# edenartlab/sd-lora-trainer

Measured on AMD Instinct MI355X. Metric: training images/sec, SDXL 1024px rank-16 LoRA, 1/2/4/8 GPU (job-parallel), higher is better.
Workload: dtype bf16

## Files before the change

sd-lora-trainer_amd/csrc/attn32.hip:

```cpp
#include "common.h"
#include "../../include/sdlt_kernels.h"
#include "attn32.h"

namespace {

constexpr float LOG2E = 1.4426950408889634f;
typedef float f32x16 __attribute__((ext_vector_type(16)));
constexpr int TILE = 64 * 128;

__device__ __forceinline__ int sw32(int row) { return (((row >> 1) & 1) << 2) | ((row >> 2) & 3); }
__device__ __forceinline__ int rmap(int rho) { return (rho & 0x13) | ((rho & 4) << 1) | ((rho & 8) >> 1); }

struct WgId { int x, y, z; };
__device__ __forceinline__ WgId xcd_wg() {
  const int gx = gridDim.x, gy = gridDim.y, n = gx * gy * gridDim.z;
  const int L = blockIdx.x + gx * (blockIdx.y + gy * blockIdx.z);
  const int k = L & 7, slot = L >> 3, q = n >> 3, r = n & 7;
  const int logical = (k < r ? k * (q + 1) : r * (q + 1) + (k - r) * q) + slot;
  WgId w;
  const int t = div_small_u(logical, gx);
  w.x = logical - t * gx;
  w.z = gridDim.z == 1 ? 0 : div_small_u(t, gy);
  w.y = t - w.z * gy;
  return w;
}

__device__ __forceinline__ void tile_dma(const bf16_t* src, int64_t ld, char* dst, int w2, int lane) {
#pragma unroll
  for (int pc = 0; pc < 4; ++pc) {
    const int piece = w2 * 4 + pc;
    const int r = piece * 8 + (lane >> 3);
    glds16(src + (int64_t)r * ld + (((lane & 7) ^ sw32(r)) << 3), dst + piece * 1024);
  }
}

template <int OFF>
__device__ __forceinline__ bf16x8 lds_b128(uint32_t a) {
  bf16x8 v;
  asm volatile("ds_read_b128 %0, %1 offset:%2" : "=v"(v) : "v"(a), "n"(OFF));
  return v;
}
template <int OFF>
__device__ __forceinline__ bf16x4 lds_tr(uint32_t a) {
  bf16x4 v;
  asm volatile("ds_read_b64_tr_b16 %0, %1 offset:%2" : "=v"(v) : "v"(a), "n"(OFF));
  return v;
}
template <int N>
__device__ __forceinline__ void wait_lgkm() { asm volatile("s_waitcnt lgkmcnt(%0)" ::"n"(N) : "memory"); }
__device__ __forceinline__ void pin(bf16x8& v) { asm volatile("" : "+v"(v)); }
__device__ __forceinline__ void pin(bf16x4& v) { asm volatile("" : "+v"(v)); }
template <int BLK>
__device__ __forceinline__ void rows_issue(bf16x8 (&f)[4], uint32_t tile, const int (&row)[4]) {
#pragma unroll
  for (int kk = 0; kk < 4; ++kk) f[kk] = lds_b128<BLK * 4096>(tile + row[kk]);
}
__device__ __forceinline__ void rows_pin(bf16x8 (&f)[4]) {
#pragma unroll
  for (int kk = 0; kk < 4; ++kk) pin(f[kk]);
}
struct TrFrag { bf16x4 v[4]; };
template <int CH>
__device__ __forceinline__ void tr_issue(TrFrag& f, uint32_t tile, const int (&t1)[2], const int (&t2)[2]) {
  f.v[0] = lds_tr<CH * 2048>(tile + t1[0]);
  f.v[1] = lds_tr<CH * 2048>(tile + t2[0]);
  f.v[2] = lds_tr<CH * 2048>(tile + t1[1]);
  f.v[3] = lds_tr<CH * 2048>(tile + t2[1]);
}
__device__ __forceinline__ void tr_pin(TrFrag& f) {
#pragma unroll
  for (int k = 0; k < 4; ++k) pin(f.v[k]);
}
__device__ __forceinline__ bf16x8 tr_get(const TrFrag& f, int db) { return __builtin_shufflevector(f.v[2 * db], f.v[2 * db + 1], 0, 1, 2, 3, 4, 5, 6, 7); }
__device__ __forceinline__ uint32_t lds_addr(const char* p) { return (uint32_t)(uintptr_t)(__attribute__((address_space(3))) const char*)p; }
__device__ __forceinline__ bf16x8 ld8(const bf16_t* p) {
  union { uint4 u; bf16x8 v; } c;
  c.u = *(const uint4*)p;
  return c.v;
}
__device__ __forceinline__ bf16x8 pack8v(const f32x16& v, int c2) {
  union { uint4 u; bf16x8 b; } c;
  c.u.x = pack2bf(v[8 * c2 + 0], v[8 * c2 + 1]); c.u.y = pack2bf(v[8 * c2 + 2], v[8 * c2 + 3]);
  c.u.z = pack2bf(v[8 * c2 + 4], v[8 * c2 + 5]); c.u.w = pack2bf(v[8 * c2 + 6], v[8 * c2 + 7]);
  return c.b;
}
__device__ __forceinline__ float half_max(float v) {
  auto r = __builtin_amdgcn_permlane32_swap(__float_as_uint(v), __float_as_uint(v), false, false);
  return fmaxf(__uint_as_float(r[0]), __uint_as_float(r[1]));
}
__device__ __forceinline__ float half_sum(float v) {
  auto r = __builtin_amdgcn_permlane32_swap(__float_as_uint(v), __float_as_uint(v), false, false);
  return __uint_as_float(r[0]) + __uint_as_float(r[1]);
}
#ifndef SDLT_A32_STORE16
#define SDLT_A32_STORE16 1
#endif
__device__ __forceinline__ void store_pair(bf16_t* p, int hl, uint2 ev, uint2 od) {
#if SDLT_A32_STORE16
  auto x = __builtin_amdgcn_permlane32_swap(ev.x, od.x, false, false);
  auto y = __builtin_amdgcn_permlane32_swap(ev.y, od.y, false, false);
  *(uint4*)p = make_uint4(x[0], y[0], x[1], y[1]);
#else
  *(uint2*)(p - 4 * hl) = ev;
  *(uint2*)(p - 4 * hl + 8) = od;
#endif
}

__device__ __forceinline__ void wait_dma_barrier() {
  asm volatile("s_waitcnt vmcnt(0)" ::: "memory");
  __syncthreads();
}

struct FragOff {
  int row[4];
  int t1[2], t2[2];
};
__device__ __forceinline__ FragOff frag_offsets(int lane) {
  FragOff f;
  const int hl = lane >> 5, c = lane & 31, rr = rmap(c);
#pragma unroll
  for (int kk = 0; kk < 4; ++kk) f.row[kk] = rr * 128 + (((2 * kk + hl) ^ sw32(rr)) << 4);
  const int g = lane >> 4, i = lane & 15;
  const int R = 8 * (g >> 1) + (i >> 2), swl = (((i >> 3) & 1) << 2) | ((g >> 1) << 1), chl = 2 * (g & 1) + ((i & 3) >> 1);
#pragma unroll
  for (int db = 0; db < 2; ++db) {
    f.t1[db] = R * 128 + (((4 * db + chl) ^ swl) << 4) + (i & 1) * 8;
    f.t2[db] = (R + 4) * 128 + (((4 * db + chl) ^ swl ^ 1) << 4) + (i & 1) * 8;
  }
  return f;
}

#define MFMA32(a, b, c) __builtin_amdgcn_mfma_f32_32x32x16_bf16(a, b, c, 0, 0, 0)

#ifndef SDLT_A32_DMA_SPLIT
#define SDLT_A32_DMA_SPLIT 1
#endif

#ifdef SDLT_ATTN32_TRACE
#define TR32_DECL(BUF_, ON_) long long* tr_ = (long long*)(BUF_); int tn_ = 0; const bool tron_ = (ON_) && tr_ != nullptr
#define TR32() do { if (tron_ && tn_ < 500) { __builtin_amdgcn_sched_barrier(0); tr_[tn_++] = clock64(); __builtin_amdgcn_sched_barrier(0); } } while (0)
#else
#define TR32_DECL(BUF_, ON_)
#define TR32() do { } while (0)
#endif

template <int KS>
__global__ __launch_bounds__(128 * KS) void attn32_fwd_kernel(const sdlt_attn_params p) {
  extern __shared__ __attribute__((aligned(16))) char smem[];
  const WgId wg = xcd_wg();
  const int b = wg.z, h = wg.y, q0 = wg.x * 64;
  const int lane = threadIdx.x & 63, wv = __builtin_amdgcn_readfirstlane(threadIdx.x >> 6);
  const int grp = wv >> 1, w2 = wv & 1, hl = lane >> 5, c = lane & 31;
  const int hc = h * 64;
  const int q = q0 + w2 * 32 + c;
  const bf16_t* Kb = (const bf16_t*)p.K + (int64_t)b * p.Nkp * p.ldk + hc;
  const bf16_t* Vb = (const bf16_t*)p.V + (int64_t)b * p.Nkp * p.ldv + hc;
  char* ring = smem + grp * (4 * TILE);
  const int ntile = p.Nk >> 6, niter = (ntile + KS - 1) / KS;
  if (grp < ntile) {
    tile_dma(Kb + (int64_t)grp * 64 * p.ldk, p.ldk, ring, w2, lane);
    tile_dma(Vb + (int64_t)grp * 64 * p.ldv, p.ldv, ring + TILE, w2, lane);
  }
  bf16x8 qf[4];
  {
    const bf16_t* qp = (const bf16_t*)p.Q + ((int64_t)b * p.Nqp + q) * p.ldq + hc + 8 * hl;
#pragma unroll
    for (int kk = 0; kk < 4; ++kk) qf[kk] = ld8(qp + 16 * kk);
  }
  const FragOff fo = frag_offsets(lane);
  float m = -1e30f, lsum = 0.f;
  f32x16 o[2];
#pragma unroll
  for (int db = 0; db < 2; ++db)
#pragma unroll
    for (int r = 0; r < 16; ++r) o[db][r] = 0.f;
  const float sl2 = p.scale * LOG2E;
  TR32_DECL(p.D, wg.x == 0 && wg.y == 0 && wg.z == 0 && threadIdx.x == 0);
  TR32();
  wait_dma_barrier();
  for (int it = 0; it < niter; ++it) {
    TR32();
    const int t = it * KS + grp;
    const char* Ks = ring + (it & 1) * (2 * TILE);
    const char* Vs = Ks + TILE;
    char* nb = ring + ((it + 1) & 1) * (2 * TILE);
    const bool more = t + KS < ntile;
#if SDLT_A32_DMA_SPLIT == 0
    if (more) {
      tile_dma(Kb + (int64_t)(t + KS) * 64 * p.ldk, p.ldk, nb, w2, lane);
      tile_dma(Vb + (int64_t)(t + KS) * 64 * p.ldv, p.ldv, nb + TILE, w2, lane);
    }
#endif
    TR32();
    if (t < ntile) {
      const uint32_t ka = lds_addr(Ks), va = lds_addr(Vs);
      bf16x8 k0f[4], k1f[4];
      TrFrag vt[4];
      rows_issue<0>(k0f, ka, fo.row);
      rows_issue<1>(k1f, ka, fo.row);
      tr_issue<0>(vt[0], va, fo.t1, fo.t2);
      tr_issue<1>(vt[1], va, fo.t1, fo.t2);
      f32x16 s[2];
#pragma unroll
      for (int blk = 0; blk < 2; ++blk)
#pragma unroll
        for (int r = 0; r < 16; ++r) s[blk][r] = 0.f;
      wait_lgkm<12>();
      rows_pin(k0f);
#pragma unroll
      for (int kk = 0; kk < 4; ++kk) s[0] = MFMA32(k0f[kk], qf[kk], s[0]);
#if SDLT_A32_DMA_SPLIT
      if (more) tile_dma(Kb + (int64_t)(t + KS) * 64 * p.ldk, p.ldk, nb, w2, lane);
#endif
      tr_issue<2>(vt[2], va, fo.t1, fo.t2);
      tr_issue<3>(vt[3], va, fo.t1, fo.t2);
      wait_lgkm<15>();
      rows_pin(k1f);
#pragma unroll
      for (int kk = 0; kk < 4; ++kk) s[1] = MFMA32(k1f[kk], qf[kk], s[1]);
#if SDLT_A32_DMA_SPLIT
      if (more) tile_dma(Vb + (int64_t)(t + KS) * 64 * p.ldv, p.ldv, nb + TILE, w2, lane);
#endif
      __builtin_amdgcn_sched_barrier(0);
      TR32();
      float tmax = s[0][0];
#pragma unroll
      for (int blk = 0; blk < 2; ++blk)
#pragma unroll
        for (int r = 0; r < 16; ++r) tmax = fmaxf(tmax, s[blk][r]);
      tmax = half_max(tmax);
      const float mn = fmaxf(m, tmax * sl2);
      const float alpha = __builtin_amdgcn_exp2f(m - mn);
      m = mn;
      float rs = 0.f;
#pragma unroll
      for (int blk = 0; blk < 2; ++blk)
#pragma unroll
        for (int r = 0; r < 16; ++r) {
          const float pv = __builtin_amdgcn_exp2f(__builtin_fmaf(s[blk][r], sl2, -mn));
          s[blk][r] = pv;
          rs += pv;
        }
      lsum = lsum * alpha + rs;
#pragma unroll
      for (int db = 0; db < 2; ++db)
#pragma unroll
        for (int r = 0; r < 16; ++r) o[db][r] *= alpha;
      __builtin_amdgcn_sched_barrier(0);
      TR32();
      wait_lgkm<0>();
#pragma unroll
      for (int ch = 0; ch < 4; ++ch) tr_pin(vt[ch]);
#pragma unroll
      for (int ch = 0; ch < 4; ++ch) {
        const bf16x8 pf = pack8v(s[ch >> 1], ch & 1);
#pragma unroll
        for (int db = 0; db < 2; ++db) o[db] = MFMA32(tr_get(vt[ch], db), pf, o[db]);
      }
    }
    TR32();
    wait_dma_barrier();
  }
  TR32();
  lsum = half_sum(lsum);
  if constexpr (KS > 1) {
    float* mg = (float*)smem + (((grp - 1) * 2 + w2) * 64 + lane) * 36;
    if (grp > 0) {
      mg[0] = m;
      mg[1] = lsum;
#pragma unroll
      for (int db = 0; db < 2; ++db)
#pragma unroll
        for (int j = 0; j < 4; ++j) *(f32x4*)(mg + 4 + db * 16 + j * 4) = (f32x4){o[db][4 * j], o[db][4 * j + 1], o[db][4 * j + 2], o[db][4 * j + 3]};
    }
    __syncthreads();
    if (grp > 0) return;
#pragma unroll
    for (int g2 = 1; g2 < KS; ++g2) {
      const float* sg = (const float*)smem + (((g2 - 1) * 2 + w2) * 64 + lane) * 36;
      const float m1 = sg[0], l1 = sg[1];
      const float mn = fmaxf(m, m1), a0 = __builtin_amdgcn_exp2f(m - mn), a1 = __builtin_amdgcn_exp2f(m1 - mn);
      m = mn;
      lsum = lsum * a0 + l1 * a1;
#pragma unroll
      for (int db = 0; db < 2; ++db)
#pragma unroll
        for (int j = 0; j < 4; ++j) {
          const f32x4 o1 = *(const f32x4*)(sg + 4 + db * 16 + j * 4);
#pragma unroll
          for (int r = 0; r < 4; ++r) o[db][4 * j + r] = o[db][4 * j + r] * a0 + o1[r] * a1;
        }
    }
  }
  const float inv = 1.f / lsum;
  if (hl == 0 && p.L) p.L[((int64_t)b * p.H + h) * p.Nq + q] = (m + log2f(lsum)) / LOG2E;
#ifndef SDLT_ATTN32_TRACE
  if (hl == 0 && p.D) p.D[((int64_t)b * p.H + h) * p.Nq + q] = 0.f;
#endif
  bf16_t* op = (bf16_t*)p.O + ((int64_t)b * p.Nqp + q) * p.ldo + hc + 8 * hl;
#pragma unroll
  for (int db = 0; db < 2; ++db)
#pragma unroll
    for (int jp = 0; jp < 2; ++jp) {
      uint2 w[2];
#pragma unroll
      for (int e = 0; e < 2; ++e) {
        const int j = 2 * jp + e;
        w[e].x = pack2bf(o[db][4 * j] * inv, o[db][4 * j + 1] * inv);
        w[e].y = pack2bf(o[db][4 * j + 2] * inv, o[db][4 * j + 3] * inv);
      }
      store_pair(op + 32 * db + 16 * jp, hl, w[0], w[1]);
    }
}

template <int KS>
__device__ __forceinline__ void attn32_dq_body(const sdlt_attn_params& p, char* smem, const int bx, const WgId wg) {
  const int b = wg.z, h = wg.y, q0 = bx * 64;
  const int lane = threadIdx.x & 63, wv = __builtin_amdgcn_readfirstlane(threadIdx.x >> 6);
  const int grp = wv >> 1, w2 = wv & 1, hl = lane >> 5, c = lane & 31;
  const int hc = h * 64;
  const int q = q0 + w2 * 32 + c;
  const bf16_t* Kb = (const bf16_t*)p.K + (int64_t)b * p.Nkp * p.ldk + hc;
  const bf16_t* Vb = (const bf16_t*)p.V + (int64_t)b * p.Nkp * p.ldv + hc;
  char* ring = smem + grp * (4 * TILE);
  const int ntile = p.Nk >> 6, niter = (ntile + KS - 1) / KS;
  if (grp < ntile) {
    tile_dma(Kb + (int64_t)grp * 64 * p.ldk, p.ldk, ring, w2, lane);
    tile_dma(Vb + (int64_t)grp * 64 * p.ldv, p.ldv, ring + TILE, w2, lane);
  }
  bf16x8 qf[4], gf[4];
  {
    const bf16_t* qp = (const bf16_t*)p.Q + ((int64_t)b * p.Nqp + q) * p.ldq + hc + 8 * hl;
    const bf16_t* gp = (const bf16_t*)p.dO + ((int64_t)b * p.Nqp + q) * p.lddo + hc + 8 * hl;
#pragma unroll
    for (int kk = 0; kk < 4; ++kk) {
      qf[kk] = ld8(qp + 16 * kk);
      gf[kk] = ld8(gp + 16 * kk);
    }
  }
  const float Lq = p.L[((int64_t)b * p.H + h) * p.Nq + q] * LOG2E;
  const float Dq = p.D[((int64_t)b * p.H + h) * p.Nq + q];
  const FragOff fo = frag_offsets(lane);
  f32x16 dq[2];
#pragma unroll
  for (int db = 0; db < 2; ++db)
#pragma unroll
    for (int r = 0; r < 16; ++r) dq[db][r] = 0.f;
  const float sl2 = p.scale * LOG2E;
  TR32_DECL(p.dK32, bx == 0 && wg.y == 0 && wg.z == 0 && threadIdx.x == 0);
  TR32();
  wait_dma_barrier();
  for (int it = 0; it < niter; ++it) {
    TR32();
    const int t = it * KS + grp;
    const char* Ks = ring + (it & 1) * (2 * TILE);
    const char* Vs = Ks + TILE;
    char* nb = ring + ((it + 1) & 1) * (2 * TILE);
    const bool more = t + KS < ntile;
#if SDLT_A32_DMA_SPLIT == 0
    if (more) {
      tile_dma(Kb + (int64_t)(t + KS) * 64 * p.ldk, p.ldk, nb, w2, lane);
      tile_dma(Vb + (int64_t)(t + KS) * 64 * p.ldv, p.ldv, nb + TILE, w2, lane);
    }
#endif
    TR32();
    if (t < ntile) {
      const uint32_t ka = lds_addr(Ks), va = lds_addr(Vs);
      bf16x8 kr[2][4], vr[2][4];
      TrFrag kt[2][2];
      rows_issue<0>(kr[0], ka, fo.row);
      rows_issue<0>(vr[0], va, fo.row);
      tr_issue<0>(kt[0][0], ka, fo.t1, fo.t2);
      tr_issue<1>(kt[0][1], ka, fo.t1, fo.t2);
#pragma unroll
      for (int blk = 0; blk < 2; ++blk) {
        f32x16 s, dp;
#pragma unroll
        for (int r = 0; r < 16; ++r) { s[r] = 0.f; dp[r] = 0.f; }
        wait_lgkm<8>();
        rows_pin(kr[blk]);
        rows_pin(vr[blk]);
#pragma unroll
        for (int kk = 0; kk < 4; ++kk) {
          s = MFMA32(kr[blk][kk], qf[kk], s);
          dp = MFMA32(vr[blk][kk], gf[kk], dp);
        }
        if (blk == 0) {
          rows_issue<1>(kr[1], ka, fo.row);
          rows_issue<1>(vr[1], va, fo.row);
        }
#if SDLT_A32_DMA_SPLIT
        if (more) {
          if (blk == 0) tile_dma(Kb + (int64_t)(t + KS) * 64 * p.ldk, p.ldk, nb, w2, lane);
          else tile_dma(Vb + (int64_t)(t + KS) * 64 * p.ldv, p.ldv, nb + TILE, w2, lane);
        }
#endif
        __builtin_amdgcn_sched_barrier(0);
        TR32();
#pragma unroll
        for (int r = 0; r < 16; ++r) {
          const float pv = __builtin_amdgcn_exp2f(__builtin_fmaf(s[r], sl2, -Lq));
          s[r] = pv * (dp[r] - Dq);
        }
        __builtin_amdgcn_sched_barrier(0);
        TR32();
        if (blk == 0) wait_lgkm<8>(); else wait_lgkm<0>();
        tr_pin(kt[blk][0]);
        tr_pin(kt[blk][1]);
#pragma unroll
        for (int c2 = 0; c2 < 2; ++c2) {
          const bf16x8 dsf = pack8v(s, c2);
#pragma unroll
          for (int db = 0; db < 2; ++db) dq[db] = MFMA32(tr_get(kt[blk][c2], db), dsf, dq[db]);
        }
        if (blk == 0) {
          tr_issue<2>(kt[1][0], ka, fo.t1, fo.t2);
          tr_issue<3>(kt[1][1], ka, fo.t1, fo.t2);
        }
        TR32();
      }
    }
    wait_dma_barrier();
  }
  TR32();
  if constexpr (KS > 1) {
    float* mg = (float*)smem + (((grp - 1) * 2 + w2) * 64 + lane) * 36;
    if (grp > 0) {
#pragma unroll
      for (int db = 0; db < 2; ++db)
#pragma unroll
        for (int j = 0; j < 4; ++j) *(f32x4*)(mg + db * 16 + j * 4) = (f32x4){dq[db][4 * j], dq[db][4 * j + 1], dq[db][4 * j + 2], dq[db][4 * j + 3]};
    }
    __syncthreads();
    if (grp > 0) return;
#pragma unroll
    for (int g2 = 1; g2 < KS; ++g2) {
      const float* sg = (const float*)smem + (((g2 - 1) * 2 + w2) * 64 + lane) * 36;
#pragma unroll
      for (int db = 0; db < 2; ++db)
#pragma unroll
        for (int j = 0; j < 4; ++j) {
          const f32x4 o1 = *(const f32x4*)(sg + db * 16 + j * 4);
#pragma unroll
          for (int r = 0; r < 4; ++r) dq[db][4 * j + r] += o1[r];
        }
    }
  }
  bf16_t* op = (bf16_t*)p.dQ + ((int64_t)b * p.Nqp + q) * p.lddq + hc + 8 * hl;
#pragma unroll
  for (int db = 0; db < 2; ++db)
#pragma unroll
    for (int jp = 0; jp < 2; ++jp) {
      uint2 w[2];
#pragma unroll
      for (int e = 0; e < 2; ++e) {
        const int j = 2 * jp + e;
        w[e].x = pack2bf(dq[db][4 * j] * p.scale, dq[db][4 * j + 1] * p.scale);
        w[e].y = pack2bf(dq[db][4 * j + 2] * p.scale, dq[db][4 * j + 3] * p.scale);
      }
      store_pair(op + 32 * db + 16 * jp, hl, w[0], w[1]);
    }
}

template <int KS>
__device__ __forceinline__ void attn32_dkdv_body(const sdlt_attn_params& p, char* smem, const int bx, const WgId wg) {
  constexpr int RING = 2 * (2 * TILE + 512);
  const int b = wg.z, h = wg.y, k0 = bx * 64;
  const int lane = threadIdx.x & 63, wv = __builtin_amdgcn_readfirstlane(threadIdx.x >> 6);
  const int grp = wv >> 1, w2 = wv & 1, hl = lane >> 5, c = lane & 31;
  const int hc = h * 64;
  const int key = k0 + w2 * 32 + c;
  const bf16_t* Qb = (const bf16_t*)p.Q + (int64_t)b * p.Nqp * p.ldq + hc;
  const bf16_t* Gb = (const bf16_t*)p.dO + (int64_t)b * p.Nqp * p.lddo + hc;
  const float* Lb = p.L + ((int64_t)b * p.H + h) * p.Nq;
  const float* Db = p.D + ((int64_t)b * p.H + h) * p.Nq;
  char* ring = smem + grp * RING;
  const int ntile = p.Nq >> 6, niter = (ntile + KS - 1) / KS;
  auto stage_q = [&](int t, char* buf) { tile_dma(Qb + (int64_t)t * 64 * p.ldq, p.ldq, buf, w2, lane); };
  auto stage_g = [&](int t, char* buf) {
    tile_dma(Gb + (int64_t)t * 64 * p.lddo, p.lddo, buf + TILE, w2, lane);
    if (lane < 16) glds16((w2 ? Db : Lb) + t * 64 + lane * 4, buf + 2 * TILE + w2 * 256);
  };
  auto stage = [&](int t, char* buf) { stage_q(t, buf); stage_g(t, buf); };
  if (grp < ntile) stage(grp, ring);
  bf16x8 kf[4], vf[4];
  {
    const bf16_t* kp = (const bf16_t*)p.K + ((int64_t)b * p.Nkp + key) * p.ldk + hc + 8 * hl;
    const bf16_t* vp = (const bf16_t*)p.V + ((int64_t)b * p.Nkp + key) * p.ldv + hc + 8 * hl;
#pragma unroll
    for (int kk = 0; kk < 4; ++kk) {
      kf[kk] = ld8(kp + 16 * kk);
      vf[kk] = ld8(vp + 16 * kk);
    }
  }
  const FragOff fo = frag_offsets(lane);
  f32x16 dk[2], dv[2];
#pragma unroll
  for (int db = 0; db < 2; ++db)
#pragma unroll
    for (int r = 0; r < 16; ++r) { dk[db][r] = 0.f; dv[db][r] = 0.f; }
  const float sl2 = p.scale * LOG2E;
  TR32_DECL(p.dK32 ? p.dK32 + 1024 : nullptr, bx == 0 && wg.y == 0 && wg.z == 0 && threadIdx.x == 0);
  TR32();
  wait_dma_barrier();
  for (int it = 0; it < niter; ++it) {
    TR32();
    const int t = it * KS + grp;
    const char* Qs = ring + (it & 1) * (2 * TILE + 512);
    const char* Gs = Qs + TILE;
    const float* Ls = (const float*)(Gs + TILE);
    const float* Ds = Ls + 64;
    char* nb = ring + ((it + 1) & 1) * (2 * TILE + 512);
    const bool more = t + KS < ntile;
#if SDLT_A32_DMA_SPLIT == 0
    if (more) stage(t + KS, nb);
#endif
    TR32();
    if (t < ntile) {
      const uint32_t qa = lds_addr(Qs), ga = lds_addr(Gs);
      bf16x8 qr[2][4], gr[2][4];
      TrFrag gt[2][2], qt[2][2];
      rows_issue<0>(qr[0], qa, fo.row);
      rows_issue<0>(gr[0], ga, fo.row);
      tr_issue<0>(gt[0][0], ga, fo.t1, fo.t2);
      tr_issue<0>(qt[0][0], qa, fo.t1, fo.t2);
#pragma unroll
      for (int blk = 0; blk < 2; ++blk) {
        f32x16 s, dp;
#pragma unroll
        for (int r = 0; r < 16; ++r) { s[r] = 0.f; dp[r] = 0.f; }
        wait_lgkm<8>();
        rows_pin(qr[blk]);
        rows_pin(gr[blk]);
#pragma unroll
        for (int kk = 0; kk < 4; ++kk) {
          s = MFMA32(qr[blk][kk], kf[kk], s);
          dp = MFMA32(gr[blk][kk], vf[kk], dp);
        }
        if (blk == 0) {
          tr_issue<1>(gt[0][1], ga, fo.t1, fo.t2);
          tr_issue<1>(qt[0][1], qa, fo.t1, fo.t2);
        } else {
          tr_issue<3>(gt[1][1], ga, fo.t1, fo.t2);
          tr_issue<3>(qt[1][1], qa, fo.t1, fo.t2);
        }
#if SDLT_A32_DMA_SPLIT
        if (more) {
          if (blk == 0) stage_q(t + KS, nb);
          else stage_g(t + KS, nb);
        }
#endif
        __builtin_amdgcn_sched_barrier(0);
        TR32();
#pragma unroll
        for (int c2 = 0; c2 < 2; ++c2) {
          const int qb = blk * 32 + c2 * 16 + 8 * hl;
          const f32x4 l0 = *(const f32x4*)(Ls + qb), l1 = *(const f32x4*)(Ls + qb + 4);
          const f32x4 d0 = *(const f32x4*)(Ds + qb), d1 = *(const f32x4*)(Ds + qb + 4);
#pragma unroll
          for (int e = 0; e < 8; ++e) {
            const float lq = (e < 4 ? l0[e & 3] : l1[e & 3]) * LOG2E, dd = e < 4 ? d0[e & 3] : d1[e & 3];
            const float pv = __builtin_amdgcn_exp2f(__builtin_fmaf(s[8 * c2 + e], sl2, -lq));
            s[8 * c2 + e] = pv;
            dp[8 * c2 + e] = pv * (dp[8 * c2 + e] - dd);
          }
        }
        __builtin_amdgcn_sched_barrier(0);
        TR32();
        wait_lgkm<8>();
        tr_pin(gt[blk][0]);
        tr_pin(qt[blk][0]);
        {
          const bf16x8 pf = pack8v(s, 0), dsf = pack8v(dp, 0);
#pragma unroll
          for (int db = 0; db < 2; ++db) {
            dv[db] = MFMA32(tr_get(gt[blk][0], db), pf, dv[db]);
            dk[db] = MFMA32(tr_get(qt[blk][0], db), dsf, dk[db]);
          }
        }
        if (blk == 0) {
          rows_issue<1>(qr[1], qa, fo.row);
          rows_issue<1>(gr[1], ga, fo.row);
          tr_issue<2>(gt[1][0], ga, fo.t1, fo.t2);
          tr_issue<2>(qt[1][0], qa, fo.t1, fo.t2);
          wait_lgkm<15>();
        } else {
          wait_lgkm<0>();
        }
        tr_pin(gt[blk][1]);
        tr_pin(qt[blk][1]);
        {
          const bf16x8 pf = pack8v(s, 1), dsf = pack8v(dp, 1);
#pragma unroll
          for (int db = 0; db < 2; ++db) {
            dv[db] = MFMA32(tr_get(gt[blk][1], db), pf, dv[db]);
            dk[db] = MFMA32(tr_get(qt[blk][1], db), dsf, dk[db]);
          }
        }
        TR32();
      }
    }
    wait_dma_barrier();
  }
  TR32();
  if constexpr (KS > 1) {
    float* mg = (float*)smem + (((grp - 1) * 2 + w2) * 64 + lane) * 68;
    if (grp > 0) {
#pragma unroll
      for (int db = 0; db < 2; ++db)
#pragma unroll
        for (int j = 0; j < 4; ++j) {
          *(f32x4*)(mg + db * 16 + j * 4) = (f32x4){dk[db][4 * j], dk[db][4 * j + 1], dk[db][4 * j + 2], dk[db][4 * j + 3]};
          *(f32x4*)(mg + 32 + db * 16 + j * 4) = (f32x4){dv[db][4 * j], dv[db][4 * j + 1], dv[db][4 * j + 2], dv[db][4 * j + 3]};
        }
    }
    __syncthreads();
    if (grp > 0) return;
#pragma unroll
    for (int g2 = 1; g2 < KS; ++g2) {
      const float* sg = (const float*)smem + (((g2 - 1) * 2 + w2) * 64 + lane) * 68;
#pragma unroll
      for (int db = 0; db < 2; ++db)
#pragma unroll
        for (int j = 0; j < 4; ++j) {
          const f32x4 a = *(const f32x4*)(sg + db * 16 + j * 4), e = *(const f32x4*)(sg + 32 + db * 16 + j * 4);
#pragma unroll
          for (int r = 0; r < 4; ++r) {
            dk[db][4 * j + r] += a[r];
            dv[db][4 * j + r] += e[r];
          }
        }
    }
  }
  const int64_t row = (int64_t)b * p.Nkp + key;
  bf16_t* kp2 = (bf16_t*)p.dK + row * p.lddk + hc + 8 * hl;
  bf16_t* vp2 = (bf16_t*)p.dV + row * p.lddv + hc + 8 * hl;
#pragma unroll
  for (int db = 0; db < 2; ++db)
#pragma unroll
    for (int jp = 0; jp < 2; ++jp) {
      uint2 wk[2], wv[2];
#pragma unroll
      for (int e = 0; e < 2; ++e) {
        const int j = 2 * jp + e;
        wk[e].x = pack2bf(dk[db][4 * j] * p.scale, dk[db][4 * j + 1] * p.scale);
        wk[e].y = pack2bf(dk[db][4 * j + 2] * p.scale, dk[db][4 * j + 3] * p.scale);
        wv[e].x = pack2bf(dv[db][4 * j], dv[db][4 * j + 1]);
        wv[e].y = pack2bf(dv[db][4 * j + 2], dv[db][4 * j + 3]);
      }
      store_pair(kp2 + 32 * db + 16 * jp, hl, wk[0], wk[1]);
      store_pair(vp2 + 32 * db + 16 * jp, hl, wv[0], wv[1]);
    }
}

template <int KS>
__global__ __launch_bounds__(128 * KS) void attn32_bwd_both_kernel(const sdlt_attn_params p) {
  extern __shared__ __attribute__((aligned(16))) char smem[];
  const int ndq = p.Nq >> 6;
  const WgId wg = xcd_wg();
  if (wg.x < ndq) attn32_dq_body<KS>(p, smem, wg.x, wg);
  else attn32_dkdv_body<KS>(p, smem, wg.x - ndq, wg);
}

template <typename F>
int set_smem32(F f, int bytes) { return sdlt_raise_smem((const void*)f, bytes); }

}

bool sdlt_attn32_ok(const sdlt_attn_params& p) {
  return p.d == 64 && !p.causal && p.Nq >= 64 && p.Nk >= 64 && (p.Nq % 64) == 0 && (p.Nk % 64) == 0 && p.Nqp >= p.Nq && p.Nkp >= p.Nk;
}

int sdlt_attn32_fwd(const sdlt_attn_params& p, int ks, hipStream_t s) {
  dim3 grid(p.Nq / 64, p.H, p.B);
#define FWD32(KS_)                                                                                           \
  do {                                                                                                       \
    const int sm = (KS_) * 4 * TILE;                                                                         \
    if (set_smem32(attn32_fwd_kernel<KS_>, sm)) SDLT_FAIL(SDLT_ERR_LAUNCH, "sdlt_attn32_fwd: LDS attribute"); \
    hipLaunchKernelGGL((attn32_fwd_kernel<KS_>), grid, dim3(128 * (KS_)), sm, s, p);                          \
  } while (0)
  if (ks >= 4) FWD32(4);
  else if (ks >= 2) FWD32(2);
  else FWD32(1);
  SDLT_CHECK_LAUNCH();
  return SDLT_OK;
}

int sdlt_attn32_bwd_both(const sdlt_attn_params& p, int ks, hipStream_t s) {
  dim3 grid(p.Nq / 64 + p.Nk / 64, p.H, p.B);
#define BWD32(KS_)                                                                                                 \
  do {                                                                                                             \
    const int sm = (KS_) * 2 * (2 * TILE + 512);                                                                   \
    if (set_smem32(attn32_bwd_both_kernel<KS_>, sm)) SDLT_FAIL(SDLT_ERR_LAUNCH, "sdlt_attn32_bwd: LDS attribute"); \
    hipLaunchKernelGGL((attn32_bwd_both_kernel<KS_>), grid, dim3(128 * (KS_)), sm, s, p);                           \
  } while (0)
  if (ks >= 4) BWD32(4);
  else if (ks >= 2) BWD32(2);
  else BWD32(1);
  SDLT_CHECK_LAUNCH();
  return SDLT_OK;
}
```

Baseline: 24.19.

## Interleave MFMA, softmax, LDS reads and DMA in attention backward kernels

Reschedules the dQ and dK/dV backward attention loops so the S and dP MFMAs, exp2 softmax, LDS fragment loads and per-piece global-to-LDS DMA are interleaved between fine-grained scheduling barriers, in place of running as separate phases. It folds the -D subtraction into the dP accumulator init, using a -D seed in dQ and a sign-flipped V with a negated dK scale in dK/dV. It also moves the L/D LDS reads into explicit early ds_read_b128 issues. The aim is to hide LDS and DMA latency behind matrix ops. The cost is more register pressure and a fragile hand schedule that relies on lgkm wait counts being correct.

Result: no change. 24.38, median of 6 (+0.8%).

```diff
diff --git a/sd-lora-trainer_amd/csrc/attn32.hip b/sd-lora-trainer_amd/csrc/attn32.hip
--- a/sd-lora-trainer_amd/csrc/attn32.hip
+++ b/sd-lora-trainer_amd/csrc/attn32.hip
@@ -313,6 +313,30 @@
     }
 }
 
+#define GAP32() __builtin_amdgcn_sched_barrier(0)
+
+template <int OFF>
+__device__ __forceinline__ f32x4 lds_f4(uint32_t a) {
+  f32x4 v;
+  asm volatile("ds_read_b128 %0, %1 offset:%2" : "=v"(v) : "v"(a), "n"(OFF));
+  return v;
+}
+__device__ __forceinline__ void pin(f32x4& v) { asm volatile("" : "+v"(v)); }
+template <int CH, int K>
+__device__ __forceinline__ void tr_issue1(TrFrag& f, uint32_t tile, const FragOff& fo) {
+  f.v[K] = lds_tr<CH * 2048>(tile + ((K & 1) ? fo.t2[K >> 1] : fo.t1[K >> 1]));
+}
+__device__ __forceinline__ void tile_dma1(const bf16_t* src, int64_t ld, char* dst, int w2, int lane, int pc) {
+  const int piece = w2 * 4 + pc;
+  const int r = piece * 8 + (lane >> 3);
+  glds16(src + (int64_t)r * ld + (((lane & 7) ^ sw32(r)) << 3), dst + piece * 1024);
+}
+__device__ __forceinline__ bf16x8 pk_frag(const uint32_t* pk) {
+  union { uint4 u; bf16x8 b; } c;
+  c.u = make_uint4(pk[0], pk[1], pk[2], pk[3]);
+  return c.b;
+}
+
 template <int KS>
 __device__ __forceinline__ void attn32_dq_body(const sdlt_attn_params& p, char* smem, const int bx, const WgId wg) {
   const int b = wg.z, h = wg.y, q0 = bx * 64;
@@ -338,8 +362,13 @@
       gf[kk] = ld8(gp + 16 * kk);
     }
   }
-  const float Lq = p.L[((int64_t)b * p.H + h) * p.Nq + q] * LOG2E;
-  const float Dq = p.D[((int64_t)b * p.H + h) * p.Nq + q];
+  const float nLq = -(p.L[((int64_t)b * p.H + h) * p.Nq + q] * LOG2E);
+  f32x16 nd;
+  {
+    const float Dq = p.D[((int64_t)b * p.H + h) * p.Nq + q];
+#pragma unroll
+    for (int r = 0; r < 16; ++r) nd[r] = -Dq;
+  }
   const FragOff fo = frag_offsets(lane);
   f32x16 dq[2];
 #pragma unroll
@@ -357,12 +386,6 @@
     const char* Vs = Ks + TILE;
     char* nb = ring + ((it + 1) & 1) * (2 * TILE);
     const bool more = t + KS < ntile;
-#if SDLT_A32_DMA_SPLIT == 0
-    if (more) {
-      tile_dma(Kb + (int64_t)(t + KS) * 64 * p.ldk, p.ldk, nb, w2, lane);
-      tile_dma(Vb + (int64_t)(t + KS) * 64 * p.ldv, p.ldv, nb + TILE, w2, lane);
-    }
-#endif
     TR32();
     if (t < ntile) {
       const uint32_t ka = lds_addr(Ks), va = lds_addr(Vs);
@@ -376,47 +399,58 @@
       for (int blk = 0; blk < 2; ++blk) {
         f32x16 s, dp;
 #pragma unroll
-        for (int r = 0; r < 16; ++r) { s[r] = 0.f; dp[r] = 0.f; }
-        wait_lgkm<8>();
+        for (int r = 0; r < 16; ++r) s[r] = 0.f;
+        if (blk == 0) wait_lgkm<8>(); else wait_lgkm<0>();
         rows_pin(kr[blk]);
         rows_pin(vr[blk]);
+        GAP32();
 #pragma unroll
         for (int kk = 0; kk < 4; ++kk) {
           s = MFMA32(kr[blk][kk], qf[kk], s);
-          dp = MFMA32(vr[blk][kk], gf[kk], dp);
-        }
-        if (blk == 0) {
-          rows_issue<1>(kr[1], ka, fo.row);
-          rows_issue<1>(vr[1], va, fo.row);
-        }
-#if SDLT_A32_DMA_SPLIT
-        if (more) {
-          if (blk == 0) tile_dma(Kb + (int64_t)(t + KS) * 64 * p.ldk, p.ldk, nb, w2, lane);
-          else tile_dma(Vb + (int64_t)(t + KS) * 64 * p.ldv, p.ldv, nb + TILE, w2, lane);
-        }
-#endif
-        __builtin_amdgcn_sched_barrier(0);
+          if (blk == 0) {
+            if (kk < 2) { kr[1][2 * kk] = lds_b128<4096>(ka + fo.row[2 * kk]); kr[1][2 * kk + 1] = lds_b128<4096>(ka + fo.row[2 * kk + 1]); }
+            else { vr[1][2 * kk - 4] = lds_b128<4096>(va + fo.row[2 * kk - 4]); vr[1][2 * kk - 3] = lds_b128<4096>(va + fo.row[2 * kk - 3]); }
+          } else {
+            if (kk == 0) { tr_issue1<2, 0>(kt[1][0], ka, fo); tr_issue1<2, 1>(kt[1][0], ka, fo); }
+            if (kk == 1) { tr_issue1<2, 2>(kt[1][0], ka, fo); tr_issue1<2, 3>(kt[1][0], ka, fo); }
+            if (kk == 2) { tr_issue1<3, 0>(kt[1][1], ka, fo); tr_issue1<3, 1>(kt[1][1], ka, fo); }
+            if (kk == 3) { tr_issue1<3, 2>(kt[1][1], ka, fo); tr_issue1<3, 3>(kt[1][1], ka, fo); }
+          }
+          GAP32();
+        }
         TR32();
 #pragma unroll
-        for (int r = 0; r < 16; ++r) {
-          const float pv = __builtin_amdgcn_exp2f(__builtin_fmaf(s[r], sl2, -Lq));
-          s[r] = pv * (dp[r] - Dq);
-        }
-        __builtin_amdgcn_sched_barrier(0);
+        for (int kk = 0; kk < 4; ++kk) {
+          dp = MFMA32(vr[blk][kk], gf[kk], kk == 0 ? nd : dp);
+#pragma unroll
+          for (int r = 4 * kk; r < 4 * kk + 4; ++r) s[r] = __builtin_amdgcn_exp2f(__builtin_fmaf(s[r], sl2, nLq));
+          if (more) {
+            if (blk == 0) tile_dma1(Kb + (int64_t)(t + KS) * 64 * p.ldk, p.ldk, nb, w2, lane, kk);
+            else tile_dma1(Vb + (int64_t)(t + KS) * 64 * p.ldv, p.ldv, nb + TILE, w2, lane, kk);
+          }
+          GAP32();
+        }
         TR32();
+#pragma unroll
+        for (int r = 0; r < 8; ++r) s[r] *= dp[r];
+        const bf16x8 ds0 = pack8v(s, 0);
         if (blk == 0) wait_lgkm<8>(); else wait_lgkm<0>();
         tr_pin(kt[blk][0]);
         tr_pin(kt[blk][1]);
-#pragma unroll
-        for (int c2 = 0; c2 < 2; ++c2) {
-          const bf16x8 dsf = pack8v(s, c2);
-#pragma unroll
-          for (int db = 0; db < 2; ++db) dq[db] = MFMA32(tr_get(kt[blk][c2], db), dsf, dq[db]);
-        }
-        if (blk == 0) {
-          tr_issue<2>(kt[1][0], ka, fo.t1, fo.t2);
-          tr_issue<3>(kt[1][1], ka, fo.t1, fo.t2);
-        }
+        GAP32();
+        dq[0] = MFMA32(tr_get(kt[blk][0], 0), ds0, dq[0]);
+#pragma unroll
+        for (int r = 8; r < 12; ++r) s[r] *= dp[r];
+        GAP32();
+        dq[1] = MFMA32(tr_get(kt[blk][0], 1), ds0, dq[1]);
+#pragma unroll
+        for (int r = 12; r < 16; ++r) s[r] *= dp[r];
+        GAP32();
+        const bf16x8 ds1 = pack8v(s, 1);
+        GAP32();
+        dq[0] = MFMA32(tr_get(kt[blk][1], 0), ds1, dq[0]);
+        dq[1] = MFMA32(tr_get(kt[blk][1], 1), ds1, dq[1]);
+        GAP32();
         TR32();
       }
     }
@@ -493,6 +527,13 @@
       vf[kk] = ld8(vp + 16 * kk);
     }
   }
+#pragma unroll
+  for (int kk = 0; kk < 4; ++kk) {
+    union { bf16x8 v; uint4 u; } n;
+    n.v = vf[kk];
+    n.u.x ^= 0x80008000u; n.u.y ^= 0x80008000u; n.u.z ^= 0x80008000u; n.u.w ^= 0x80008000u;
+    vf[kk] = n.v;
+  }
   const FragOff fo = frag_offsets(lane);
   f32x16 dk[2], dv[2];
 #pragma unroll
@@ -508,18 +549,23 @@
     const int t = it * KS + grp;
     const char* Qs = ring + (it & 1) * (2 * TILE + 512);
     const char* Gs = Qs + TILE;
-    const float* Ls = (const float*)(Gs + TILE);
-    const float* Ds = Ls + 64;
     char* nb = ring + ((it + 1) & 1) * (2 * TILE + 512);
     const bool more = t + KS < ntile;
-#if SDLT_A32_DMA_SPLIT == 0
-    if (more) stage(t + KS, nb);
-#endif
     TR32();
     if (t < ntile) {
       const uint32_t qa = lds_addr(Qs), ga = lds_addr(Gs);
+      const uint32_t la = lds_addr(Gs + TILE) + 32 * hl, da = la + 256;
       bf16x8 qr[2][4], gr[2][4];
       TrFrag gt[2][2], qt[2][2];
+      f32x4 lv[2][4], dd[2][4];
+#define LD_ISSUE(BLK_)                                                                  \
+  do {                                                                                  \
+    lv[BLK_][0] = lds_f4<(BLK_) * 128>(la);      lv[BLK_][1] = lds_f4<(BLK_) * 128 + 16>(la); \
+    lv[BLK_][2] = lds_f4<(BLK_) * 128 + 64>(la); lv[BLK_][3] = lds_f4<(BLK_) * 128 + 80>(la); \
+    dd[BLK_][0] = lds_f4<(BLK_) * 128>(da);      dd[BLK_][1] = lds_f4<(BLK_) * 128 + 16>(da); \
+    dd[BLK_][2] = lds_f4<(BLK_) * 128 + 64>(da); dd[BLK_][3] = lds_f4<(BLK_) * 128 + 80>(da); \
+  } while (0)
+      LD_ISSUE(0);
       rows_issue<0>(qr[0], qa, fo.row);
       rows_issue<0>(gr[0], ga, fo.row);
       tr_issue<0>(gt[0][0], ga, fo.t1, fo.t2);
@@ -527,78 +573,81 @@
 #pragma unroll
       for (int blk = 0; blk < 2; ++blk) {
         f32x16 s, dp;
-#pragma unroll
-        for (int r = 0; r < 16; ++r) { s[r] = 0.f; dp[r] = 0.f; }
+        float lq[16];
         wait_lgkm<8>();
         rows_pin(qr[blk]);
         rows_pin(gr[blk]);
 #pragma unroll
+        for (int j = 0; j < 4; ++j) { pin(lv[blk][j]); pin(dd[blk][j]); }
+#pragma unroll
+        for (int r = 0; r < 16; ++r) { s[r] = 0.f; dp[r] = dd[blk][r >> 2][r & 3]; }
+        GAP32();
+#pragma unroll
         for (int kk = 0; kk < 4; ++kk) {
           s = MFMA32(qr[blk][kk], kf[kk], s);
+#pragma unroll
+          for (int r = 4 * kk; r < 4 * kk + 4; ++r) lq[r] = lv[blk][kk][r & 3] * LOG2E;
+          gt[blk][1].v[kk] = blk == 0 ? lds_tr<2048>(ga + ((kk & 1) ? fo.t2[kk >> 1] : fo.t1[kk >> 1])) : lds_tr<3 * 2048>(ga + ((kk & 1) ? fo.t2[kk >> 1] : fo.t1[kk >> 1]));
+          GAP32();
+        }
+#pragma unroll
+        for (int kk = 0; kk < 4; ++kk) {
           dp = MFMA32(gr[blk][kk], vf[kk], dp);
-        }
-        if (blk == 0) {
-          tr_issue<1>(gt[0][1], ga, fo.t1, fo.t2);
-          tr_issue<1>(qt[0][1], qa, fo.t1, fo.t2);
-        } else {
-          tr_issue<3>(gt[1][1], ga, fo.t1, fo.t2);
-          tr_issue<3>(qt[1][1], qa, fo.t1, fo.t2);
-        }
-#if SDLT_A32_DMA_SPLIT
-        if (more) {
-          if (blk == 0) stage_q(t + KS, nb);
-          else stage_g(t + KS, nb);
-        }
-#endif
-        __builtin_amdgcn_sched_barrier(0);
+#pragma unroll
+          for (int r = 4 * kk; r < 4 * kk + 4; ++r) s[r] = __builtin_amdgcn_exp2f(__builtin_fmaf(s[r], sl2, -lq[r]));
+          qt[blk][1].v[kk] = blk == 0 ? lds_tr<2048>(qa + ((kk & 1) ? fo.t2[kk >> 1] : fo.t1[kk >> 1])) : lds_tr<3 * 2048>(qa + ((kk & 1) ? fo.t2[kk >> 1] : fo.t1[kk >> 1]));
+          if (more) {
+            if (blk == 0) tile_dma1(Qb + (int64_t)(t + KS) * 64 * p.ldq, p.ldq, nb, w2, lane, kk);
+            else tile_dma1(Gb + (int64_t)(t + KS) * 64 * p.lddo, p.lddo, nb + TILE, w2, lane, kk);
+          }
+          GAP32();
+        }
+        if (more && blk == 1 && lane < 16) glds16((w2 ? Db : Lb) + (t + KS) * 64 + lane * 4, nb + 2 * TILE + w2 * 256);
         TR32();
 #pragma unroll
-        for (int c2 = 0; c2 < 2; ++c2) {
-          const int qb = blk * 32 + c2 * 16 + 8 * hl;
-          const f32x4 l0 = *(const f32x4*)(Ls + qb), l1 = *(const f32x4*)(Ls + qb + 4);
-          const f32x4 d0 = *(const f32x4*)(Ds + qb), d1 = *(const f32x4*)(Ds + qb + 4);
-#pragma unroll
-          for (int e = 0; e < 8; ++e) {
-            const float lq = (e < 4 ? l0[e & 3] : l1[e & 3]) * LOG2E, dd = e < 4 ? d0[e & 3] : d1[e & 3];
-            const float pv = __builtin_amdgcn_exp2f(__builtin_fmaf(s[8 * c2 + e], sl2, -lq));
-            s[8 * c2 + e] = pv;
-            dp[8 * c2 + e] = pv * (dp[8 * c2 + e] - dd);
-          }
-        }
-        __builtin_amdgcn_sched_barrier(0);
-        TR32();
+        for (int r = 0; r < 8; ++r) dp[r] *= s[r];
+        const bf16x8 pf0 = pack8v(s, 0), dsf0 = pack8v(dp, 0);
         wait_lgkm<8>();
         tr_pin(gt[blk][0]);
         tr_pin(qt[blk][0]);
-        {
-          const bf16x8 pf = pack8v(s, 0), dsf = pack8v(dp, 0);
-#pragma unroll
-          for (int db = 0; db < 2; ++db) {
-            dv[db] = MFMA32(tr_get(gt[blk][0], db), pf, dv[db]);
-            dk[db] = MFMA32(tr_get(qt[blk][0], db), dsf, dk[db]);
-          }
-        }
+        GAP32();
+        TR32();
+        dv[0] = MFMA32(tr_get(gt[blk][0], 0), pf0, dv[0]);
+        dp[8] *= s[8]; dp[9] *= s[9];
+        GAP32();
+        dk[0] = MFMA32(tr_get(qt[blk][0], 0), dsf0, dk[0]);
+        dp[10] *= s[10]; dp[11] *= s[11];
+        GAP32();
+        dv[1] = MFMA32(tr_get(gt[blk][0], 1), pf0, dv[1]);
+        dp[12] *= s[12]; dp[13] *= s[13];
+        GAP32();
+        dk[1] = MFMA32(tr_get(qt[blk][0], 1), dsf0, dk[1]);
+        dp[14] *= s[14]; dp[15] *= s[15];
+        GAP32();
+        const bf16x8 pf1 = pack8v(s, 1), dsf1 = pack8v(dp, 1);
+        wait_lgkm<0>();
+        tr_pin(gt[blk][1]);
+        tr_pin(qt[blk][1]);
+        GAP32();
+        dv[0] = MFMA32(tr_get(gt[blk][1], 0), pf1, dv[0]);
+        if (blk == 0) { LD_ISSUE(1); }
+        GAP32();
+        dk[0] = MFMA32(tr_get(qt[blk][1], 0), dsf1, dk[0]);
+        if (blk == 0) rows_issue<1>(qr[1], qa, fo.row);
+        GAP32();
+        dv[1] = MFMA32(tr_get(gt[blk][1], 1), pf1, dv[1]);
+        if (blk == 0) rows_issue<1>(gr[1], ga, fo.row);
+        GAP32();
+        dk[1] = MFMA32(tr_get(qt[blk][1], 1), dsf1, dk[1]);
         if (blk == 0) {
-          rows_issue<1>(qr[1], qa, fo.row);
-          rows_issue<1>(gr[1], ga, fo.row);
           tr_issue<2>(gt[1][0], ga, fo.t1, fo.t2);
           tr_issue<2>(qt[1][0], qa, fo.t1, fo.t2);
-          wait_lgkm<15>();
-        } else {
-          wait_lgkm<0>();
-        }
-        tr_pin(gt[blk][1]);
-        tr_pin(qt[blk][1]);
-        {
-          const bf16x8 pf = pack8v(s, 1), dsf = pack8v(dp, 1);
-#pragma unroll
-          for (int db = 0; db < 2; ++db) {
-            dv[db] = MFMA32(tr_get(gt[blk][1], db), pf, dv[db]);
-            dk[db] = MFMA32(tr_get(qt[blk][1], db), dsf, dk[db]);
-          }
-        }
+        }
+        GAP32();
         TR32();
       }
+#undef LD_ISSUE
+      wait_lgkm<0>();
     }
     wait_dma_barrier();
   }
@@ -635,6 +684,7 @@
   const int64_t row = (int64_t)b * p.Nkp + key;
   bf16_t* kp2 = (bf16_t*)p.dK + row * p.lddk + hc + 8 * hl;
   bf16_t* vp2 = (bf16_t*)p.dV + row * p.lddv + hc + 8 * hl;
+  const float nsc = -p.scale;
 #pragma unroll
   for (int db = 0; db < 2; ++db)
 #pragma unroll
@@ -643,8 +693,8 @@
 #pragma unroll
       for (int e = 0; e < 2; ++e) {
         const int j = 2 * jp + e;
-        wk[e].x = pack2bf(dk[db][4 * j] * p.scale, dk[db][4 * j + 1] * p.scale);
-        wk[e].y = pack2bf(dk[db][4 * j + 2] * p.scale, dk[db][4 * j + 3] * p.scale);
+        wk[e].x = pack2bf(dk[db][4 * j] * nsc, dk[db][4 * j + 1] * nsc);
+        wk[e].y = pack2bf(dk[db][4 * j + 2] * nsc, dk[db][4 * j + 3] * nsc);
         wv[e].x = pack2bf(dv[db][4 * j], dv[db][4 * j + 1]);
         wv[e].y = pack2bf(dv[db][4 * j + 2], dv[db][4 * j + 3]);
       }
```
